# zraorg/ZRA

Measured on AMD Instinct MI355X. Metric: compress + RA-decompress GiB/s, 16 GiB @ 64 KiB frames, 1/2/4/8 MI355X, higher is better.
Workload: dtype u8

## Files before the change

zra_amd/csrc/zra_encode.hip:

```cpp
#include <cstdio>
#include <unistd.h>
#include "zra_engine.h"
#include "zra_dev.h"
#include "zra_format.h"
#include "zra_env.h"
#include <algorithm>
#include <cstdlib>
#include <cstring>
#include <vector>

extern "C" __global__ void zra_mf_kernel(ZraEncArgs a, uint32_t block, uint32_t only, uint32_t onlySlot, uint32_t perWave);
extern "C" __global__ void zra_mf_opt_kernel(ZraEncArgs a, uint32_t block, uint32_t only, uint32_t onlySlot, uint32_t perWave);
extern "C" __global__ void zra_mf_dfast_ls_kernel(ZraEncArgs a, uint32_t block, uint32_t only, uint32_t onlySlot);
extern "C" __global__ void zra_mf_hc_kernel(ZraEncArgs a, uint32_t block, uint32_t only, uint32_t onlySlot);
extern "C" __global__ void zra_mf_fast_kernel(ZraEncArgs a, uint32_t block, uint32_t perWave);
extern "C" __global__ void zra_mf_dfast_kernel(ZraEncArgs a, uint32_t block, uint32_t only, uint32_t onlySlot);
extern "C" __global__ void zra_mf_dfast_fl_kernel(ZraEncArgs a, ZraFlagArgs g, uint32_t block, uint32_t only, uint32_t onlySlot);
extern "C" __global__ void zra_entropy_kernel(ZraEncArgs a, uint32_t block);
extern "C" __global__ void zra_entropy_front_kernel(ZraEncArgs a, uint32_t block);
extern "C" __global__ void zra_entropy_back_kernel(ZraEncArgs a, uint32_t block);
extern "C" __global__ void zra_ent_chain_kernel(ZraEncArgs a);
extern "C" __global__ void zra_ent_chain5_kernel(ZraEncArgs a);

using namespace zra_dev;
// ... 356 lines not shown
  encCounters_ = dCnt; encCountersBytes_ = 4 * (4 + 8 * (size_t)nSuper + 4 * (size_t)(nSuper * subsPerSuper));

  ZraEncArgs base{};
  base.in = dIn; base.inSize = inSize; base.frameSize = frameSize; base.checksum = checksum ? 1 : 0;
  base.full = full; base.tail = tail;
  dbgSeqStride_ = seqStride; dbgB_ = (uint32_t)SBIG;
  base.tableStride = tableWords; base.seqStride = seqStride; base.litStride = litStride; base.slotStride = slotStride;
  base.mfTele = (uint64_t*)(encScan_.as<uint8_t>() + cntCore);
  base.entWorkStride = entWorkStride;
  base.entPrio = 1;
  base.entSubFrames = SB; base.slotRing = (uint32_t)slotRing; base.readyStamp = 1u;
  const uint32_t shL = 1, shS = 3, dupLog = 8;
  base.mfFilter = shL | (shS << 4) | (dupLog << 8);
  const uint32_t hl = std::max(full.hashLog, tail.hashLog), cl = std::max(full.chainLog, tail.chainLog);
  const size_t filterBytes = (8u << dupLog) + (((size_t)1 << hl) >> shL) / 8 + (((size_t)1 << cl) >> shS) / 8;

  static const int lsEnv = env_int("ZRA_MF_LS", 1);
  const uint32_t lsBytes = (uint32_t)((std::min<uint64_t>(frameSize, inSize) + 64 + 63) & ~63ull);
  const uint32_t lsPerCu = (uint32_t)((160u << 10) / (lsBytes + filterBytes));
  static const int lsMaxEnv = env_int("ZRA_MF_LS_MAX", -1);
  bool useLs = lsEnv != 0 && full.strategy == 2 && lsPerCu >= 1 &&
               nFramesTotal <= (lsMaxEnv >= 0 ? (uint64_t)lsMaxEnv : (uint64_t)lsPerCu * (uint64_t)numCUs_);
  if (useLs && lsAttr_ == 0) {
    const bool okA = hipFuncSetAttribute((const void*)zra_mf_dfast_ls_kernel, hipFuncAttributeMaxDynamicSharedMemorySize, 160 << 10) == hipSuccess;
    if (!okA) (void)hipGetLastError();
    lsAttr_ = okA ? 1 : -1;
  }
  if (lsAttr_ < 0) useLs = false;

  static const int flEnv = env_int("ZRA_MF_FLAGS", 1);
  const bool useFlagsWave = flEnv != 0 && !useLs && full.strategy == 2;
  ZraFlagArgs fw{};
  if (useFlagsWave) {
    fw.flagStride = ((((uint64_t)std::min<uint64_t>(frameSize, inSize) + 511) / 512) * 128 + 255) & ~255ull;
    if (!mfFlags_.reserve((size_t)nSlots * fw.flagStride)) return zerr(64);
    fw.flags = mfFlags_.as<uint8_t>(); fw.ldsWords = (uint32_t)(filterBytes / 4);
    fw.spanBytes = 768;
    static const int epEnv = env_int("ZRA_MF_EPOCH", 4);
    const uint32_t ibMax = 32u - (uint32_t)__builtin_clz((uint32_t)std::max<uint64_t>(2, std::min<uint64_t>(frameSize, inSize)) - 1u);
    fw.epochBits = (uint32_t)std::max(0, std::min(epEnv, (int)(32u - ibMax) - 10));
  }
  const size_t spanLds = fw.spanBytes ? fw.spanBytes + 16 + (fw.spanBytes / 64 + 1) * 16 : 0;

  size_t evNext = 0;
  auto ev = [&]() -> hipEvent_t {
    if (evNext == evPool_.size()) { hipEvent_t e = nullptr; if (hipEventCreate(&e) != hipSuccess) return nullptr; evPool_.push_back(e); }
    return evPool_[evNext++];
  };
  std::vector<std::pair<hipEvent_t, hipEvent_t>> mfSpans, entSpans;
  static const bool traceOn = env_set("ZRA_ENC_TRACE");
  hipEvent_t superDone[2] = {nullptr, nullptr};
  { hipEvent_t e0 = ev(); if (!e0) return zerr(1); HIPCHK(hipEventRecord(e0, stream_)); HIPCHK(hipStreamWaitEvent(stream2_, e0, 0)); }

  for (uint64_t S = 0; S < nSuper; S++) {
    const uint64_t F0 = S * SBIG;
    const uint32_t n = (uint32_t)std::min<uint64_t>(SBIG, nFramesTotal - F0);
    const int c = (int)(S % nCtx);
    EncCtx& x = encCtx_[c];
    ZraEncArgs a = base;
    a.firstFrame = (uint32_t)F0; a.nFrames = n;
    a.tables = sh.tables.as<uint32_t>(); a.lits = sh.lits.as<uint8_t>(); a.slots = sh.slots.as<uint8_t>(); a.entWork = sh.work.as<uint8_t>();
    a.seqs = x.seqs.as<uint64_t>();
    a.state = x.misc.as<ZraEncFrameState>();
    a.blockOut = (ZraEncBlockOut*)(x.misc.as<uint8_t>() + (size_t)SBIG * sizeof(ZraEncFrameState));
    a.contentCk = x.ck.as<uint32_t>();
    a.sizes = x.sizes.as<uint64_t>();
    a.mfQueue = dPerSuper + 8 * S; a.mfStarted = a.mfQueue + 1;
    uint32_t* const entQ = dPerSub + 4 * S * subsPerSuper;
    a.mfDone = entQ + 3 * subsPerSuper;
    if (superDone[c]) HIPCHK(hipStreamWaitEvent(stream_, superDone[c], 0));
    HIPCHK(hipMemsetAsync(a.blockOut, 0, (size_t)n * sizeof(ZraEncBlockOut), stream_));
    hipEvent_t m0 = ev(), m1 = ev();
    if (!m0 || !m1) return zerr(1);
    HIPCHK(hipEventRecord(m0, stream_));
    const uint32_t mfGrid = std::min<uint32_t>(n, nSlots);
// ... 209 lines not shown
```

zra_amd/csrc/zra_encode_mf.hip:

```cpp
#include "zra_dev.h"
#include "zra_kernels.h"
#include "zra_encode_wave.h"

using namespace zra_dev;
using namespace zra_wave;

#ifdef ZRA_MF_PROFILE
__device__ unsigned long long zra_mf_prof[24];
#define PROF_DECL u64 pt_[20]; for (int k_ = 0; k_ < 20; k_++) pt_[k_] = 0; u64 pl_ = __builtin_amdgcn_s_memtime();
#define PROF(k) { __builtin_amdgcn_s_waitcnt(0); const u64 n_ = __builtin_amdgcn_s_memtime(); pt_[k] += n_ - pl_; pl_ = n_; }
#define PROF_CNT(k) { pt_[k]++; }
#define PROF_END { if (lane == 0) for (int k_ = 0; k_ < 20; k_++) atomicAdd(&zra_mf_prof[k_], pt_[k_]); }
#elif defined(ZRA_MF_MARK)
#define PROF_DECL
#define PROF(k) asm volatile("; ZMARK " #k);
#define PROF_CNT(k)
#define PROF_END
#else
#define PROF_DECL
#define PROF(k)
#define PROF_CNT(k)
#define PROF_END
#endif

// ... 343 lines not shown
      tS = (((p4 >> ib) & keep) | epoch) << ib;
    }
    if (MLS == 5) bS = (u32)(((v << 24) * 889523592379ULL) >> shS);
    else if (MLS == 6) bS = (u32)(((v << 16) * 227718039650203ULL) >> shS);
    else if (MLS == 7) bS = (u32)(((v << 8) * 58295818150454627ULL) >> shS);
    else bS = p4 >> shS;
  }
};

struct __attribute__((packed, aligned(1))) quad_u { u32 x, y, z, w; };
__device__ __forceinline__ uint4 ld128(const u8* p) { const quad_u q = *(const quad_u*)p; return make_uint4(q.x, q.y, q.z, q.w); }

struct LeanLds {
  u8* dup; u32 dupSlots; u32* bmL; u32* bmS; u32 shL, shS;
  u8* span; u8* spanFlg; u32 spanBytes;
  __device__ __forceinline__ void markL(u32 b) const { const u32 g = b >> shL; atomicOr(&bmL[g >> 5], 1u << (g & 31)); }
  __device__ __forceinline__ void markS(u32 b) const { const u32 g = b >> shS; atomicOr(&bmS[g >> 5], 1u << (g & 31)); }
};

#ifdef ZRA_MF_NT
#define TLD(p) __builtin_nontemporal_load(p)
#define TST(p, v) __builtin_nontemporal_store((u32)(v), p)
#elif defined(ZRA_MF_SC1ST)
#ifdef ZRA_MF_SC1LD
#define TLD(p) __hip_atomic_load((p), __ATOMIC_RELAXED, __HIP_MEMORY_SCOPE_AGENT)
#else
#define TLD(p) (*(p))
#endif
#define TST(p, v) __hip_atomic_store((p), (u32)(v), __ATOMIC_RELAXED, __HIP_MEMORY_SCOPE_AGENT)
#else
#define TLD(p) (*(p))
#define TST(p, v) (*(p) = (v))
#endif
__device__ __forceinline__ u32 df_flags_at(const u8* flg, u32 p) {
  const u8* const w = flg + (size_t)(p >> 6) * 16 + ((p & 63u) >> 3);
  const u32 b = p & 7u;
  return 0x05u | (((w[0] >> b) & 1u) << 1) | (((w[8] >> b) & 1u) << 3);
}
#define ZRA_DF_EPOCH_BITS 4u
template <u32 MLS, bool FLAGS>
__device__ u32 mf_dfast_lean(const ZraEncParams& P, u32* HL, u32* HS, const u8* src, u32 bs, u32 be, u32* rep, u64* seqs, u32* nOut,
                             const LeanLds& W, int lane, u32 ib, const u8* flgIn, u32 epoch = 0) {
  const u8* const flg = FLAGS ? flgIn : nullptr;
  DfHash<MLS, FLAGS ? ZRA_DF_EPOCH_BITS : 0u> H; H.init(P.hashLog, P.chainLog, ib, FLAGS ? rfl(epoch) : 0u);
  const u32 idxMask = ~H.tagMask;
  bs = rfl(bs); be = rfl(be);
  u32 o1 = rfl(rep[0]), o2 = rfl(rep[1]), saved;
  u32 anchor = bs, nseq = 0;
  const u32 ilimit = be >= 8 ? be - 8 : 0;
  u32 ip = mf_prologue(bs, o1, o2, saved);
  u32 sqLo = 0, sqHi = 0;
  u32* const dL = (u32*)W.dup; u32* const dS = dL + W.dupSlots;
  const u32 dmask = W.dupSlots - 1;
  for (u32 i = (u32)lane; i < 2 * W.dupSlots; i += 64) dL[i] = 0;
  u32 dupRound = 0;
  u32* const bmL = W.bmL; u32* const bmS = W.bmS;
  PROF_DECL
  auto emit = [&](u32 ll, u32 ml, u32 offVal) {
    const u64 q = (u64)ll | ((u64)ml << 20) | ((u64)offVal << 40);
    sqLo = wlane(sqLo, (u32)q, nseq & 63); sqHi = wlane(sqHi, (u32)(q >> 32), nseq & 63);
    nseq++;
    if ((nseq & 63) == 0) seqs[nseq - 64 + (u32)lane] = (u64)sqLo | ((u64)sqHi << 32);
  };
  auto insert_slow = [&](u32 pos, bool doL, bool doS) {
    if (lane == 0) {
      const u32 fx = flg ? df_flags_at(flg, pos) : 0x0Fu;
      u32 bl, bs_, tl, ts; H.both(ld64(src + pos), bl, bs_, tl, ts);
      if (doL && (fx & 2)) { TST(HL + bl, (pos + 1) | tl); W.markL(bl); }
      if (doS && (fx & 8)) { TST(HS + bs_, (pos + 1) | ts); W.markS(bs_); }
    }
  };
  const bool useSpan = FLAGS && W.spanBytes != 0;
  u32 sBase = 0, sEnd = 0;
  auto span_fill = [&](u32 at) {
    const u32 mis = (u32)((uintptr_t)(src + at) & 15u);
    const u32 base = rfl(at - min(at, mis));
    const u32 len = min(W.spanBytes, be - base);
    const u32 o = 16u * (u32)lane;
    if (o + 16 <= len) lds_write128(W.span + o, ld128(src + base + o));
    else if (o < len) { for (u32 k = o; k < len; k++) lds_write8(W.span + k, src[base + k]); }
    if (flg) {
      const u32 l2 = (u32)lane, w0 = base >> 6;
      if (l2 <= (W.spanBytes >> 6) && (w0 + l2) * 64u < be) lds_write128(W.spanFlg + 16u * l2, *(const uint4*)(flg + 16u * (size_t)(w0 + l2)));
    }
    __builtin_amdgcn_wave_barrier();
    sBase = base; sEnd = base + len;
  };
  while (ip < ilimit) {
    const u32 wip = ip, run = ip - anchor;
    u32 s = 1, nAct;
    if (run < 256) nAct = min(min(64u, 256u - run), ilimit - ip);
    else { s = (run >> 8) + 1; nAct = min(64u, min((256 * s - run + s - 1) / s, (ilimit - ip + s - 1) / s)); }
    bool active = (u32)lane < nAct;
    const u32 p = wip + (u32)lane * s;
    u64 v8; u32 bflags;
    if (useSpan && s == 1) {
      if (wip < sBase || wip + nAct + 7 > sEnd) span_fill(wip);
      const u32 r = p - sBase;
      v8 = active ? *(const lds_u64u_t*)(W.span + r) : 0;
      bflags = 0x0Fu;
      if (flg && active) {
        const u8* const w = W.spanFlg + ((p >> 6) - (sBase >> 6)) * 16u + ((p & 63u) >> 3);
        const u32 b = p & 7u;
        bflags = 0x05u | (((lds_read8(w) >> b) & 1u) << 1) | (((lds_read8(w + 8) >> b) & 1u) << 3);
      }
    } else {
      v8 = active ? ld64(src + p) : 0;
      bflags = (flg && active) ? df_flags_at(flg, p) : 0x0Fu;
    }
    u32 repFor = o1;
    bool rv = active && o1 > 0 && p + 1 >= o1;
    u32 repVal = rv ? ld32(src + p + 1 - o1) : 0;
    PROF(0) PROF_CNT(12)
    u32 bL, bS, tL, tS; H.both(v8, bL, bS, tL, tS);
    if (nAct > 1) {
      bool pL = active, pS = active;
      u64 mates = 0;
      for (;;) {
        dupRound++;
        const u32 key = (dupRound << 6) | (63u - (u32)lane);
        if (pL) atomicMax(&dL[bL & dmask], key);
        if (pS) atomicMax(&dS[bS & dmask], key);
        __builtin_amdgcn_wave_barrier();
        const u32 wl = pL ? 63u - (lds_read32(&dL[bL & dmask]) & 63u) : (u32)lane;
        const u32 ws = pS ? 63u - (lds_read32(&dS[bS & dmask]) & 63u) : (u32)lane;
        __builtin_amdgcn_wave_barrier();
        const u32 obL = (u32)__shfl((int)bL, (int)wl, 64), obS = (u32)__shfl((int)bS, (int)ws, 64);
        const bool lostL = wl != (u32)lane, lostS = ws != (u32)lane;
        const bool sameL = lostL && obL == bL, sameS = lostS && obS == bS;
        mates |= __ballot(sameL || sameS);
        pL = lostL && !sameL; pS = lostS && !sameS;
        PROF_CNT(17)
        if (!__ballot(pL || pS)) break;
      }
      if (mates) { nAct = (u32)__builtin_ctzll(mates); active = (u32)lane < nAct; }
    }
    PROF(1)
    const u32 gL = bL >> W.shL, gS = bS >> W.shS;
    const u32 wL = gL >> 5, wS = gS >> 5, qL = 1u << (gL & 31), qS = 1u << (gS & 31);
    u32 mL = 0, mS = 0;
    if (active) {
      const bool needL = (bflags & 1) && (bmL[wL] & qL) != 0, needS = (bflags & 4) && (bmS[wS] & qS) != 0;
      const u32 rL = needL ? TLD(HL + bL) : 0u, rS = needS ? TLD(HS + bS) : 0u;
      mL = ((rL & H.tagMask) == tL) ? (rL & idxMask) : 0u;
      mS = ((rS & H.tagMask) == tS) ? (rS & idxMask) : 0u;
    }
    PROF(2)
    u64 LH = __ballot(active && mL > 1);
    u64 SH = __ballot(active && mS > 1);
    const u32 valL = (p + 1) | tL, valS = (p + 1) | tS;
    const u32 v8s = (u32)(v8 >> 8);
    const u64 AM = nAct >= 64 ? ~0ull : (bit64(nAct) - 1);
    u64 RH = __ballot(rv && repVal == v8s);
    u32 repOld = 0, repOldFor = 0xFFFFFFFFu; u64 ROV = 0;
    u64 RV = __ballot(rv);
    PROF(3)
    u32 cur = 0;
    for (;;) {
      if (repFor != o1) {
        rv = active && o1 > 0 && p + 1 >= o1;
        repVal = rv ? ld32(src + p + 1 - o1) : 0; repFor = o1;
        RH = __ballot(rv && repVal == v8s); RV = __ballot(rv);
      }
      const u64 live = AM & (~0ull << cur);
      const u64 hm = (RH | LH | SH) & live;
      if (!hm) {
        if (lane_in(live)) { if (bflags & 2) { TST(HL + bL, valL); atomicOr(&bmL[wL], qL); } if (bflags & 8) { TST(HS + bS, valS); atomicOr(&bmS[wS], qS); } }
        ip = wip + nAct * s; PROF(4)
        break;
      }
      const u32 f = (u32)__builtin_ctzll(hm);
      u64 mkL = live & ((bit64(f) << 1) - 1), mkS = mkL;
      const u32 top = wip + f * s;
      const bool isRep = (RH >> f) & 1, isLong = (LH >> f) & 1;
      ip = top;
      u32 m, known, offVal = 1;
      u32 vneed = 0, mS2 = 0; bool dual = false;
      if (isRep) { ip = top + 1; m = ip - o1; known = 4; }
      else if (isLong) { m = bcast(mL, f) - 1; known = 0; vneed = 8; }
      else if (s == 1 && f + 1 < nAct) {
        mkL |= bit64(f + 1);
        if ((LH >> (f + 1)) & 1) { m = bcast(mL, f + 1) - 1; ip = top + 1; known = 0; vneed = 8; dual = true; mS2 = bcast(mS, f) - 1; }
        else { m = bcast(mS, f) - 1; known = 0; vneed = 4; }
      } else {
        bool hit3; u32 m3;
        {
          PROF_CNT(15)
          if (rfl(ld32(src + bcast(mS, f) - 1)) != bcast((u32)v8, f)) { SH &= ~bit64(f); continue; }
          if (lane_in(mkL) && (bflags & 2)) { TST(HL + bL, valL); atomicOr(&bmL[wL], qL); }
          if (lane_in(mkS) && (bflags & 8)) { TST(HS + bS, valS); atomicOr(&bmS[wS], qS); }
          mkL = 0; mkS = 0;
          u32 m3v = 0; bool h3v = false;
          if (lane == 0) {
            const u64 v9 = ld64(src + top + 1);
            const u32 f3 = flg ? df_flags_at(flg, top + 1) : 0x0Fu;
            u32 b3, bx, t3, tx; H.both(v9, b3, bx, t3, tx);
            const u32 r3 = (f3 & 1) ? TLD(HL + b3) : 0u;
            m3v = ((r3 & H.tagMask) == t3) ? (r3 & idxMask) : 0u;
            if (f3 & 2) { TST(HL + b3, (top + 2) | t3); W.markL(b3); }
            h3v = m3v > 1 && ld64(src + m3v - 1) == v9;
          }
          hit3 = __ballot(h3v) & 1; m3 = bcast(m3v, 0);
        }
        if (hit3) { m = m3 - 1; ip = top + 1; known = 8; }
        else { m = bcast(mS, f) - 1; known = 4; }
      }
      PROF(5)
#ifdef ZRA_MF_PAD_SALU
      { u32 sd_ = nseq;
#pragma unroll
        for (int k_ = 0; k_ < ZRA_MF_PAD_SALU; k_++) asm volatile("s_add_u32 %0, %0, 1" : "+s"(sd_) :: "scc"); }
#endif
#ifdef ZRA_MF_PAD_VALU
      { u32 vd_ = (u32)lane;
#pragma unroll
        for (int k_ = 0; k_ < ZRA_MF_PAD_VALU; k_++) asm volatile("v_add_u32 %0, %0, 1" : "+v"(vd_)); }
#endif
      u32 off = ip - m;
      const u32 l16 = (u32)lane & 15u;
      const bool sec = dual && (u32)lane >= 16 && (u32)lane < 32;
      const u32 fa = sec ? top + 8 * l16 : ip + known + 8 * (u32)lane, fb = sec ? mS2 + 8 * l16 : m + known + 8 * (u32)lane;
      const bool fv = ((u32)lane < 16 || sec) && fa + 8 <= be;
      const u64 xa = fv ? ld64(src + fa) : 0, xb = fv ? ld64(src + fb) : 0;
      const u32 lim = isRep ? 0u : min(ip - anchor, m);
      u32 ya = 0, yb = 1;
      if (lim) { const bool bv = (u32)lane < lim; ya = bv ? src[ip - 1 - lane] : 0u; yb = bv ? src[m - 1 - lane] : 1u; }
      u32 rnext = 0; bool rvn = false;
      if (!isRep) { rvn = active && p + 1 >= off; rnext = rvn ? ld32(src + p + 1 - off) : 0; }
      u32 ml;
      bool redo = false;
      {
        const u64 d = xa ^ xb;
// ... 5 lines not shown
        if (clean) ml = known + 8 * l + bcast(eq, l);
        else ml = known + wave_count_eq(src, ip + known, m + known, be, lane);
        if (dual) {
          const u64 stopS = (stopAll >> 16) & 0xFFFFull;
          const u32 lS = stopS ? (u32)__builtin_ctzll(stopS) : 16u;
          const bool cleanS = stopS && ((fvAll >> (16 + lS)) & 1);
          const u32 mlS = cleanS ? 8 * lS + bcast(eq, 16 + lS) : wave_count_eq(src, top, mS2, be, lane);
          if (mlS < 4) { SH &= ~bit64(f); continue; }
          if (ml < 8) { m = mS2; ip = top; ml = mlS; off = ip - m; redo = true; }
        } else if (ml < vneed) {
          if (isLong) LH &= ~bit64(f); else SH &= ~bit64(f);
          continue;
        }
      }
      PROF(6)
      if (!isRep) {
        u32 back = 0;
        if (redo) {
          back = wave_count_back(src, ip, m, anchor, lane);
          rvn = active && p + 1 >= off; rnext = rvn ? ld32(src + p + 1 - off) : 0;
        } else if (lim) {
          const u64 bad = ~__ballot(ya == yb);
          back = bad ? (u32)__builtin_ctzll(bad) : wave_count_back(src, ip, m, anchor, lane);
        }
        ip -= back; ml += back;
        o2 = o1; o1 = off; offVal = off + 3;
        repOld = repVal; ROV = RV; repOldFor = repFor;
        repVal = rnext; repFor = off; RV = __ballot(rvn); RH = __ballot(rvn && rnext == v8s);
      }
      emit(ip - anchor, ml, offVal);
      ip += ml; anchor = ip;
      PROF(7) PROF_CNT(13)
      if (ip > ilimit) {
        if (lane_in(mkL) && (bflags & 2)) { TST(HL + bL, valL); atomicOr(&bmL[wL], qL); }
        if (lane_in(mkS) && (bflags & 8)) { TST(HS + bS, valS); atomicOr(&bmS[wS], qS); }
        break;
      }
      const u32 relE = ip - wip;
      const bool in2 = s == 1 && f + 2 < nAct;
      const bool inE = s == 1 && relE - 1 < nAct;
      const bool inI = s == 1 && relE < nAct;
      if (in2) { mkL |= bit64(f + 2); mkS |= bit64(f + 2); }
      if (s == 1 && relE - 2 < nAct) mkL |= bit64(relE - 2);
      if (inE) mkS |= bit64(relE - 1);
      if (lane_in(mkL) && (bflags & 2)) { TST(HL + bL, valL); atomicOr(&bmL[wL], qL); }
      if (lane_in(mkS) && (bflags & 8)) { TST(HS + bS, valS); atomicOr(&bmS[wS], qS); }
      u32 here = 0, there = 1;
      const bool thereIn = inI && repOldFor == o2 && ((ROV >> (relE - 1)) & 1);
      if (in2 && inE && (o2 == 0 || thereIn)) {
        if (o2) { here = bcast((u32)v8, relE); there = bcast(repOld, relE - 1); }
      } else {
        PROF_CNT(14)
        const u32 ipos = lane < 2 ? top + 2 : lane == 2 ? ip - 2 : lane == 3 ? ip - 1 : lane == 4 ? ip : ip - o2;
        const u64 x = lane < 6 ? ld64(src + ipos) : 0;
        const u32 fx = (flg && lane < 4) ? df_flags_at(flg, ipos) : 0x0Fu;
        const bool wr = (lane & 1) ? (fx & 8) != 0 : (fx & 2) != 0;
        u32 xbL, xbS, xtL, xtS; H.both(x, xbL, xbS, xtL, xtS);
        u32* const tp = (lane & 1) ? HS + xbS : HL + xbL;
        const u32 tv = (ipos + 1) | ((lane & 1) ? xtS : xtL);
        if (lane < 4 && wr) { if (lane & 1) W.markS(xbS); else W.markL(xbL); }
        if (!in2 && lane < 2 && wr) TST(tp, tv);
        asm volatile("" ::: "memory");
        const u64 later = (s == 1 && relE - 2 < nAct ? 0ull : 4ull) | (inE ? 0ull : 8ull);
        if (lane_in(later) && wr) TST(tp, tv);
        here = bcast((u32)x, 4); there = o2 ? bcast((u32)x, 5) : here + 1;
        if (o2 == 0) { here = 0; there = 1; }
      }
      PROF(8)
      if (here == there) {
        for (;;) {
          PROF_CNT(16)
          const u32 rl = wave_count_eq(src, ip + 4, ip + 4 - o2, be, lane) + 4;
          const u32 t = o2; o2 = o1; o1 = t;
          insert_slow(ip, true, true);
          emit(0, rl, 1);
          ip += rl; anchor = ip;
          if (!(ip <= ilimit && o2 > 0)) break;
          if (rfl(ld32(src + ip)) != rfl(ld32(src + ip - o2))) break;
        }
      }
      PROF(9)
      if (s != 1 || ip >= wip + nAct || ip >= ilimit) break;
      cur = ip - wip;
    }
  }
  if (nseq & 63) { if ((u32)lane < (nseq & 63)) seqs[(nseq & ~63u) + (u32)lane] = (u64)sqLo | ((u64)sqHi << 32); }
  PROF(10) PROF_END
  rep[0] = o1 ? o1 : saved; rep[1] = o2 ? o2 : saved;
  *nOut = nseq;
// ... 326 lines not shown
    O.hashLog3 = P.minMatch == 3 ? min(17u, P.windowLog) : 0;
    O.hash3 = chainT + ((size_t)1 << P.chainLog);
    O.o = (ZraOptState*)(O.hash3 + (O.hashLog3 ? (size_t)1 << O.hashLog3 : 0));
    O.idxShift = st->idxShift;
    ntu = ntu0;
    { const u32 cur = bs + 1 + O.idxShift; if (cur > ntu + 384) { const u32 d = cur - ntu - 384; ntu = cur - (d < 192 ? d : 192); } }
    O.nextToUpdate = ntu;
    if (P.strategy == 9 && O.o->litLengthSum == 0 && bs == 0 && ntu == 1 && be - bs > 1024) {
      u32 tmpRep[3] = {rep[0], rep[1], rep[2]};
      (void)O.parse(src, bs, be, tmpRep, E, true);
      O.idxShift += be - bs;
      O.nextToUpdate = 1 + O.idxShift;
      O.upscale_stats();
    }
    lastLL = O.parse(src, bs, be, rep, E, false);
    ntu = O.nextToUpdate;
    st->idxShift = O.idxShift;
  } else if (P.strategy == 1) lastLL = mf_fast(P, hashT, src, bs, be, rep, E);
  else if (P.strategy == 2) lastLL = mf_dfast_serial(P, hashT, chainT, src, bs, be, rep, E);
  else {
    HC H; H.hashT = hashT; H.chainT = chainT; H.hlog = P.hashLog; H.mls = P.minMatch < 4 ? 4 : P.minMatch > 6 ? 6 : P.minMatch;
    H.chainSize = 1u << P.chainLog; H.cmask = H.chainSize - 1; H.searchLog = P.searchLog; H.nextToUpdate = ntu;
    H.windowLog = P.windowLog;
    H.bt = P.strategy == 6;
    lastLL = mf_lazy(H, src, bs, be, rep, E, P.strategy == 6 ? 2 : (int)P.strategy - 3);
    ntu = H.nextToUpdate;
  }
  st->nextToUpdate = ntu; st->insEnd = ntu;
  bo->nbSeq = E.n; bo->lastLL = lastLL;
  bo->rep[0] = rep[0]; bo->rep[1] = rep[1]; bo->rep[2] = rep[2];
}

struct DfBlock { u64 a; u64 m; };
__device__ __forceinline__ DfBlock df_block_load(const u8* src, u32 fsize, const u8* flg, u32 blk, bool haveMasks, int lane) {
  DfBlock B; B.a = 0; B.m = 0;
  const u32 c = blk * 512 + 8 * (u32)lane;
  if (c + 8 <= fsize) B.a = ld64(src + c);
  else if (c < fsize) B.a = ld64_safe(src + c, src + fsize);
  if (haveMasks && lane < 16) B.m = *(const u64*)(flg + (size_t)blk * 128 + 8 * (u32)lane);
  return B;
}
__device__ __forceinline__ void df_later_flags(const u8* src, u32 fsize, u32 hlog, u32 clog, u32 mls, u32* lds, u32 ldsWords, u8* flg, int lane) {
  if (fsize < 8) return;
  const u32 lastPos = fsize - 8;
  const u32 bmWords = ldsWords - 128;
  u32 npLog = 0;
  while ((((1u << hlog) + (1u << clog)) >> npLog) > bmWords * 32) npLog++;
  const u32 hlogP = hlog - npLog, clogP = clog - npLog;
  u32* const cnt = lds; u32* const bmL = lds + 128; u32* const bmS = bmL + ((1u << hlogP) >> 5);
  const u64 primeS = mls == 5 ? 889523592379ULL : mls == 6 ? 227718039650203ULL : 58295818150454627ULL;
  const u32 shV = 64 - 8 * min(mls, 7u);
  const u32 nBlk = lastPos / 512 + 1;
  const u32 srcLane = (u32)lane >> 3, sh = ((u32)lane & 7u) * 8;
  for (u32 pass = 0; pass < (1u << npLog); pass++) {
    for (u32 i = (u32)lane; i < 128 + ((1u << hlogP) >> 5) + ((1u << clogP) >> 5); i += 64) lds[i] = 0;
    __builtin_amdgcn_fence(__ATOMIC_ACQ_REL, "workgroup");
    const bool hm = pass != 0;
    DfBlock B0 = df_block_load(src, fsize, flg, nBlk - 1, hm, lane), B1{0, 0};
    u64 above = nBlk * 512 < fsize ? ld64_safe(src + nBlk * 512, src + fsize) : 0;
    for (u32 blk = nBlk; blk-- > 0;) {
      if (blk >= 1) B1 = df_block_load(src, fsize, flg, blk - 1, hm, lane);
      const u32 aLo = (u32)B0.a, aHi = (u32)(B0.a >> 32);
      u64 outM = 0;
#pragma unroll 1
      for (u32 kk = 0; kk < 4; kk++) {
        if (blk * 512 + (6 - 2 * kk) * 64 > lastPos) continue;
        u32 iLw[2], iSw[2]; bool pLw[2], pSw[2];
#pragma unroll
        for (int h = 0; h < 2; h++) {
          const u32 k = 7 - 2 * kk - h;
          const u32 p = blk * 512 + k * 64 + (u32)lane;
          const bool act = p <= lastPos;
          const u32 ci = 8 * k + srcLane;
          const u32 c0l = (u32)__builtin_amdgcn_ds_bpermute((int)(4 * ci), (int)aLo), c0h = (u32)__builtin_amdgcn_ds_bpermute((int)(4 * ci), (int)aHi);
          u32 c1l = (u32)__builtin_amdgcn_ds_bpermute((int)(4 * ((ci + 1) & 63)), (int)aLo), c1h = (u32)__builtin_amdgcn_ds_bpermute((int)(4 * ((ci + 1) & 63)), (int)aHi);
          if (ci == 63) { c1l = (u32)above; c1h = (u32)(above >> 32); }
          const u64 c0 = (u64)c0l | ((u64)c0h << 32), c1 = (u64)c1l | ((u64)c1h << 32);
          const u64 v = sh ? (c0 >> sh) | (c1 << (64 - sh)) : c0;
          const u32 bL = (u32)((v * 0xCF1BBCDCB7A56463ULL) >> (64 - hlog));
          const u32 bS = mls <= 4 ? ((u32)v * 2654435761u) >> (32 - clog) : (u32)(((v << shV) * primeS) >> (64 - clog));
          pLw[h] = act && (bL >> hlogP) == pass; pSw[h] = act && (bS >> clogP) == pass;
          iLw[h] = bL & ((1u << hlogP) - 1); iSw[h] = bS & ((1u << clogP) - 1);
        }
        u32 seenL[2], seenS[2], cL[2], cS[2];
#pragma unroll
        for (int h = 0; h < 2; h++) {
          const u32 iL = iLw[h], iS = iSw[h], sL = iL & 255u, sS = 256u + (iS & 255u);
          const bool pL = pLw[h], pS = pSw[h];
          seenL[h] = pL ? lds_read32(&bmL[iL >> 5]) : 0u; seenS[h] = pS ? lds_read32(&bmS[iS >> 5]) : 0u;
          if (pL) atomicAdd(&cnt[sL >> 2], 1u << (8 * (sL & 3)));
          if (pS) atomicAdd(&cnt[sS >> 2], 1u << (8 * (sS & 3)));
          __builtin_amdgcn_wave_barrier();
          cL[h] = pL ? lds_read32(&cnt[sL >> 2]) : 0u;
          cS[h] = pS ? lds_read32(&cnt[sS >> 2]) : 0u;
          __builtin_amdgcn_wave_barrier();
          if (pL) { atomicSub(&cnt[sL >> 2], 1u << (8 * (sL & 3))); atomicOr(&bmL[iL >> 5], 1u << (iL & 31)); }
          if (pS) { atomicSub(&cnt[sS >> 2], 1u << (8 * (sS & 3))); atomicOr(&bmS[iS >> 5], 1u << (iS & 31)); }
          __builtin_amdgcn_wave_barrier();
        }
#pragma unroll
        for (int h = 0; h < 2; h++) {
          const u32 k = 7 - 2 * kk - h;
          if (blk * 512 + k * 64 > lastPos) continue;
          const u32 iL = iLw[h], iS = iSw[h], sL = iL & 255u, sS = iS & 255u;
          const u64 mL = __ballot(((seenL[h] >> (iL & 31)) & 1u) || ((cL[h] >> (8 * (sL & 3))) & 255u) > 1);
          const u64 mS = __ballot(((seenS[h] >> (iS & 31)) & 1u) || ((cS[h] >> (8 * (sS & 3))) & 255u) > 1);
          if ((u32)lane == 2 * k) outM = mL;
          if ((u32)lane == 2 * k + 1) outM = mS;
        }
      }
      if (lane < 16) *(u64*)(flg + (size_t)blk * 128 + 8 * (u32)lane) = outM | B0.m;
      above = (u64)bcast(aLo, 0) | ((u64)bcast(aHi, 0) << 32);
      B0 = B1;
    }
    __builtin_amdgcn_fence(__ATOMIC_RELEASE, "agent");
    __builtin_amdgcn_fence(__ATOMIC_ACQUIRE, "agent");
  }
}
template <bool FLAGS, bool LSRC = false>
__device__ __forceinline__ void mf_dfast_body(const ZraEncArgs& a, u32 block, u32 only, u32 onlySlot, const ZraFlagArgs* g = nullptr) {
  const int lane = threadIdx.x;
  extern __shared__ u32 dynLds[];
  LeanLds W;
  W.shL = a.mfFilter & 15; W.shS = (a.mfFilter >> 4) & 15; W.dupSlots = 1u << ((a.mfFilter >> 8) & 15);
  u32* const fltLds = LSRC ? dynLds + (a.mfFilter >> 16) * 16 : dynLds;
  W.dup = (u8*)fltLds;
  W.bmL = fltLds + 2 * W.dupSlots;
  W.span = nullptr; W.spanFlg = nullptr; W.spanBytes = 0;
  if (FLAGS && g && g->spanBytes) { W.spanBytes = g->spanBytes; W.span = (u8*)(fltLds + g->ldsWords); W.spanFlg = W.span + g->spanBytes + 16; }
  const bool persistent = a.mfQueue != nullptr;
  const bool tele = persistent && a.mfTele != nullptr;
  u64* const tl = tele ? a.mfTele + ZRA_TELE_HEAD + 4 * (size_t)min(blockIdx.x, ZRA_TELE_WAVES - 1u) : nullptr;
  if (tele && lane == 0) {
    const u32 hw = __builtin_amdgcn_s_getreg((31 << 11) | 4);
    const u32 xcc = __builtin_amdgcn_s_getreg((3 << 11) | 20) & 7u;
    const u64 tc0 = __builtin_readcyclecounter(), tr0 = wall_clock64();
    const u32 key = (xcc << 8) | (((hw >> 13) & 7u) << 5) | (((hw >> 12) & 1u) << 4) | ((hw >> 8) & 15u);
    atomicAdd((unsigned long long*)&a.mfTele[32 + key], 1ull << (16u * ((hw >> 4) & 3u)));
    atomicAdd((unsigned long long*)&a.mfTele[8 + xcc], 1ull);
    atomicMax((unsigned long long*)&a.mfTele[4], ~tr0);
    atomicMax((unsigned long long*)&a.mfTele[6], tr0);
    tl[0] = tc0; tl[1] = tr0; tl[2] = xcc; tl[3] = 0;
  }
  if (persistent && a.mfStarted && lane == 0) atomicAdd(a.mfStarted, 1u);
  const u32 epochBits = (FLAGS && g && persistent) ? min(g->epochBits, ZRA_DF_EPOCH_BITS) : 0u;
  u32 epochCtr = 0;
  for (;;) {
    u32 f = only == 0xFFFFFFFFu ? blockIdx.x : only;
    if (persistent) {
      u32 t = 0;
      if (lane == 0) t = atomicAdd(a.mfQueue, 1u);
      f = rfl(t);
      if (f >= a.nFrames) {
        if (tele && lane == 0) {
          const u64 tc1 = __builtin_readcyclecounter(), tr1 = wall_clock64();
          const u64 tc0 = tl[0], tr0 = tl[1];
          const u32 xcc = (u32)tl[2] & 7u;
          atomicAdd((unsigned long long*)&a.mfTele[0], tc1 - tc0);
          atomicAdd((unsigned long long*)&a.mfTele[1], tr1 - tr0);
          atomicAdd((unsigned long long*)&a.mfTele[2], 1ull);
          atomicMax((unsigned long long*)&a.mfTele[3], tr1 - tr0);
          atomicMax((unsigned long long*)&a.mfTele[5], tr1);
// ... 7 lines not shown
    }
#ifdef ZRA_MF_PROFILE
    const u64 kt0_ = __builtin_amdgcn_s_memtime();
#endif
    bool mine = true;
    {
      const u64 fstart = (u64)(a.firstFrame + f) * a.frameSize;
      const ZraEncParams& Pf = (a.inSize - fstart < a.frameSize) ? a.tail : a.full;
      if (Pf.strategy != 2) mine = false;
    }
    MfFrame F;
    bool keepTables = false; u32 epoch = 0;
    if (epochBits && mine) {
      const u64 fstart = (u64)(a.firstFrame + f) * a.frameSize;
      const bool fullFrame = a.inSize - fstart >= a.frameSize;
      if (!fullFrame) epochCtr = 0;
      epoch = epochCtr & ((1u << epochBits) - 1u);
      keepTables = epoch != 0;
      epochCtr = fullFrame ? epochCtr + 1 : 0;
    }
    if (mine && mf_frame_setup(a, block, lane, F, f, persistent ? blockIdx.x : only == 0xFFFFFFFFu ? f : onlySlot, false, keepTables)) {
#ifdef ZRA_MF_PROFILE
      __builtin_amdgcn_s_waitcnt(0);
      if (lane == 0) atomicAdd(&zra_mf_prof[20], __builtin_amdgcn_s_memtime() - kt0_);
#endif
      const u32 wordsL = ((1u << F.P->hashLog) >> W.shL) / 32, wordsS = ((1u << F.P->chainLog) >> W.shS) / 32;
      W.bmS = W.bmL + wordsL;
      u32 rep[3] = {F.st->rep[0], F.st->rep[1], F.st->rep[2]};
      u32 lastLL, nseq = 0;
      const u32 ib = 32 - __builtin_clz(F.fsize - 1);
      const u8* flg = nullptr;
      if (FLAGS && g && g->flags && block == 0 && persistent) {
        u8* const fw = g->flags + (size_t)blockIdx.x * g->flagStride;
        df_later_flags(F.src, F.fsize, F.P->hashLog, F.P->chainLog, F.P->minMatch, fltLds, g->ldsWords, fw, lane);
        flg = fw;
      }
      {
        const u32 fill = block == 0 ? 0u : 0xFFFFFFFFu;
        for (u32 i = lane; i < wordsL + wordsS; i += 64) W.bmL[i] = fill;
        __builtin_amdgcn_fence(__ATOMIC_ACQ_REL, "workgroup");
      }
      const u8* srcP = F.src;
      if (LSRC) {
        u8* const ls = (u8*)dynLds;
        const u32 n16 = F.fsize >> 4;
        for (u32 i = (u32)lane; i < n16; i += 64) *(uint4*)(ls + 16 * i) = ld128(F.src + 16 * i);
        for (u32 i = (n16 << 4) + (u32)lane; i < F.fsize; i += 64) ls[i] = F.src[i];
        ls[F.fsize + (u32)lane] = 0;
        __builtin_amdgcn_fence(__ATOMIC_RELEASE, "workgroup");
        __builtin_amdgcn_wave_barrier();
        __builtin_amdgcn_fence(__ATOMIC_ACQUIRE, "workgroup");
        srcP = ls;
      }
      switch (F.P->minMatch) {
        case 5: lastLL = mf_dfast_lean<5, FLAGS>(*F.P, F.hashT, F.chainT, srcP, F.bs, F.be, rep, F.seqs, &nseq, W, lane, ib, flg, epoch); break;
        case 6: lastLL = mf_dfast_lean<6, FLAGS>(*F.P, F.hashT, F.chainT, srcP, F.bs, F.be, rep, F.seqs, &nseq, W, lane, ib, flg, epoch); break;
        case 7: lastLL = mf_dfast_lean<7, FLAGS>(*F.P, F.hashT, F.chainT, srcP, F.bs, F.be, rep, F.seqs, &nseq, W, lane, ib, flg, epoch); break;
        default: lastLL = mf_dfast_lean<4, FLAGS>(*F.P, F.hashT, F.chainT, srcP, F.bs, F.be, rep, F.seqs, &nseq, W, lane, ib, flg, epoch); break;
      }
      if (lane == 0) {
        F.bo->nbSeq = nseq; F.bo->lastLL = lastLL; F.bo->skip = 0;
        F.bo->rep[0] = rep[0]; F.bo->rep[1] = rep[1]; F.bo->rep[2] = rep[2];
      }
#ifdef ZRA_MF_PROFILE
      __builtin_amdgcn_s_waitcnt(0);
      if (lane == 0) { atomicAdd(&zra_mf_prof[21], __builtin_amdgcn_s_memtime() - kt0_); atomicAdd(&zra_mf_prof[22], 1ull); }
#endif
// ... 114 lines not shown
```

zra_amd/csrc/zra_kernels.h:

```cpp
#pragma once
#include <stdint.h>
#include <stddef.h>

#ifndef ZRA_HUF_FRAMES
#define ZRA_HUF_FRAMES 2
#endif
#define ZRA_DEC_TBL_LL 0u
#define ZRA_DEC_TBL_ML 512u
#define ZRA_DEC_TBL_OF 1024u
#define ZRA_DEC_TBL_WORDS 1280u
#define ZRA_LDS_TBL_LL 0u
#define ZRA_LDS_TBL_ML 1024u
#define ZRA_LDS_TBL_OF 2048u
#define ZRA_LDS_TBL_WORDS 2304u
#define ZRA_CHAIN_LDS_FRAMES 59u
#define ZRA_CHAIN_RING_WORDS 36u

struct ZraDecFrame {
  uint32_t blkPos, produced, done;
  uint32_t hufValid, hufMaxBits, hufNSym, hufX2;
  uint32_t llValid, mlValid, ofValid, llLog, mlLog, ofLog, ofShare;
  uint32_t rep[3];
  uint32_t fcsLo, fcsHi, fcsHave, hasChecksum, bigWindow;
  uint32_t bpos, bsize, blast;
// ... 146 lines not shown
  uint32_t* contentCk;
  uint64_t* sizes;
  uint32_t* mfQueue;
  uint32_t* mfStarted;
  uint32_t* mfDone;
  uint32_t* entQueue;
  uint32_t* entDone;
  uint32_t* scanDone;
  uint32_t* gatherJ;
  uint32_t* gQueue;
  uint32_t* gCopied;
  uint32_t* gatherDone;
  uint32_t* pipeAbort;
  uint64_t* offsets;
  uint64_t* running;
  uint8_t* gBody;
  uint8_t* gEntries;
  uint64_t* gSizesOut;
  uint32_t entSubFrames;
  uint32_t slotRing;
  uint32_t readyStamp;
  uint32_t entPrio;
  uint64_t* mfTele;
  ZraEntRec* entRec;
};
#define ZRA_TELE_CUKEYS 2048u
#define ZRA_TELE_HEAD (32u + ZRA_TELE_CUKEYS)
#define ZRA_TELE_WAVES 8192u
#define ZRA_TELE_ENT (ZRA_TELE_HEAD + 4u * ZRA_TELE_WAVES)
#define ZRA_TELE_WORDS (ZRA_TELE_ENT + 8u + ZRA_TELE_CUKEYS)
struct ZraFlagArgs {
  uint8_t* flags; uint64_t flagStride; uint32_t ldsWords;
  uint32_t spanBytes;
  uint32_t epochBits;
};
```

Measured before the change: 20.37.

## Add forward-pass bucket flags to skip useless hash reads and reuse span LDS

The flag pre-pass now runs in both directions. Besides the existing 'later' bits that gate hash-table writes, it produces 'earlier' bits that gate hash-table reads, which halves the flag stride's density (32 bytes per 64 positions). The match-finder packs the four flag bits into one word per position in LDS and skips global hash loads when no earlier occurrence can exist. Post-match inserts now read bytes and flags from the LDS span instead of global memory, and the span size shrinks. The cost is a second flag pass over each frame and more flag memory traffic, traded against fewer random hash-table reads.

```diff
diff --git a/zra_amd/csrc/zra_encode.hip b/zra_amd/csrc/zra_encode.hip
--- a/zra_amd/csrc/zra_encode.hip
+++ b/zra_amd/csrc/zra_encode.hip
@@ -412,15 +412,20 @@
   const bool useFlagsWave = flEnv != 0 && !useLs && full.strategy == 2;
   ZraFlagArgs fw{};
   if (useFlagsWave) {
-    fw.flagStride = ((((uint64_t)std::min<uint64_t>(frameSize, inSize) + 511) / 512) * 128 + 255) & ~255ull;
+    static const int earlierEnv = env_int("ZRA_MF_EARLIER", 1);
+    fw.earlier = earlierEnv != 0 ? 1u : 0u;
+    fw.flagStride = ((((uint64_t)std::min<uint64_t>(frameSize, inSize) + 511) / 512) * 256 + 255) & ~255ull;
+    static const int spanComplEnv = env_int("ZRA_MF_SPAN_COMPL", 1);
+    fw.spanCompl = spanComplEnv != 0 ? 1u : 0u;
     if (!mfFlags_.reserve((size_t)nSlots * fw.flagStride)) return zerr(64);
     fw.flags = mfFlags_.as<uint8_t>(); fw.ldsWords = (uint32_t)(filterBytes / 4);
-    fw.spanBytes = 768;
+    if (!fw.earlier) HIPCHK(hipMemsetAsync(fw.flags, 0xFF, (size_t)nSlots * fw.flagStride, stream_));
+    fw.spanBytes = 640;
     static const int epEnv = env_int("ZRA_MF_EPOCH", 4);
     const uint32_t ibMax = 32u - (uint32_t)__builtin_clz((uint32_t)std::max<uint64_t>(2, std::min<uint64_t>(frameSize, inSize)) - 1u);
     fw.epochBits = (uint32_t)std::max(0, std::min(epEnv, (int)(32u - ibMax) - 10));
   }
-  const size_t spanLds = fw.spanBytes ? fw.spanBytes + 16 + (fw.spanBytes / 64 + 1) * 16 : 0;
+  const size_t spanLds = fw.spanBytes ? fw.spanBytes + 16 + (fw.spanBytes / 64 + 1) * 32 : 0;
 
   size_t evNext = 0;
   auto ev = [&]() -> hipEvent_t {
diff --git a/zra_amd/csrc/zra_encode_mf.hip b/zra_amd/csrc/zra_encode_mf.hip
--- a/zra_amd/csrc/zra_encode_mf.hip
+++ b/zra_amd/csrc/zra_encode_mf.hip
@@ -399,10 +399,17 @@
 #define TLD(p) (*(p))
 #define TST(p, v) (*(p) = (v))
 #endif
+#define DF_WL 0x00000001u
+#define DF_WS 0x00000100u
+#define DF_RL 0x00010000u
+#define DF_RS 0x01000000u
+#define DF_ALL 0x01010101u
+template <bool EARLIER>
 __device__ __forceinline__ u32 df_flags_at(const u8* flg, u32 p) {
-  const u8* const w = flg + (size_t)(p >> 6) * 16 + ((p & 63u) >> 3);
-  const u32 b = p & 7u;
-  return 0x05u | (((w[0] >> b) & 1u) << 1) | (((w[8] >> b) & 1u) << 3);
+  const u8* const w = flg + (size_t)(p >> 6) * 32 + ((p & 63u) >> 3);
+  u32 d = (u32)w[0] | ((u32)w[8] << 8);
+  if (EARLIER) d |= ((u32)w[16] << 16) | ((u32)w[24] << 24); else d |= 0xFFFF0000u;
+  return (d >> (p & 7u)) & DF_ALL;
 }
 #define ZRA_DF_EPOCH_BITS 4u
 template <u32 MLS, bool FLAGS>
@@ -431,10 +438,10 @@
   };
   auto insert_slow = [&](u32 pos, bool doL, bool doS) {
     if (lane == 0) {
-      const u32 fx = flg ? df_flags_at(flg, pos) : 0x0Fu;
+      const u32 fx = flg ? df_flags_at<false>(flg, pos) : DF_ALL;
       u32 bl, bs_, tl, ts; H.both(ld64(src + pos), bl, bs_, tl, ts);
-      if (doL && (fx & 2)) { TST(HL + bl, (pos + 1) | tl); W.markL(bl); }
-      if (doS && (fx & 8)) { TST(HS + bs_, (pos + 1) | ts); W.markS(bs_); }
+      if (doL && (fx & DF_WL)) { TST(HL + bl, (pos + 1) | tl); W.markL(bl); }
+      if (doS && (fx & DF_WS)) { TST(HS + bs_, (pos + 1) | ts); W.markS(bs_); }
     }
   };
   const bool useSpan = FLAGS && W.spanBytes != 0;
@@ -442,13 +449,18 @@
   auto span_fill = [&](u32 at) {
     const u32 mis = (u32)((uintptr_t)(src + at) & 15u);
     const u32 base = rfl(at - min(at, mis));
-    const u32 len = min(W.spanBytes, be - base);
+    const u32 len = min(W.spanBytes & ~1u, be - base);
     const u32 o = 16u * (u32)lane;
     if (o + 16 <= len) lds_write128(W.span + o, ld128(src + base + o));
     else if (o < len) { for (u32 k = o; k < len; k++) lds_write8(W.span + k, src[base + k]); }
     if (flg) {
       const u32 l2 = (u32)lane, w0 = base >> 6;
-      if (l2 <= (W.spanBytes >> 6) && (w0 + l2) * 64u < be) lds_write128(W.spanFlg + 16u * l2, *(const uint4*)(flg + 16u * (size_t)(w0 + l2)));
+      if (l2 <= (W.spanBytes >> 6) && (w0 + l2) * 64u < be) {
+        const uint4 wl = *(const uint4*)(flg + 32u * (size_t)(w0 + l2)), el = *(const uint4*)(flg + 32u * (size_t)(w0 + l2) + 16);
+        auto mix = [](u32 a, u32 b, u32 c, u32 d, u32 j) { return ((a >> (8 * j)) & 255u) | (((b >> (8 * j)) & 255u) << 8) | (((c >> (8 * j)) & 255u) << 16) | ((d >> (8 * j)) << 24); };
+        lds_write128(W.spanFlg + 32u * l2, make_uint4(mix(wl.x, wl.z, el.x, el.z, 0), mix(wl.x, wl.z, el.x, el.z, 1), mix(wl.x, wl.z, el.x, el.z, 2), mix(wl.x, wl.z, el.x, el.z, 3)));
+        lds_write128(W.spanFlg + 32u * l2 + 16u, make_uint4(mix(wl.y, wl.w, el.y, el.w, 0), mix(wl.y, wl.w, el.y, el.w, 1), mix(wl.y, wl.w, el.y, el.w, 2), mix(wl.y, wl.w, el.y, el.w, 3)));
+      }
     }
     __builtin_amdgcn_wave_barrier();
     sBase = base; sEnd = base + len;
@@ -465,15 +477,11 @@
       if (wip < sBase || wip + nAct + 7 > sEnd) span_fill(wip);
       const u32 r = p - sBase;
       v8 = active ? *(const lds_u64u_t*)(W.span + r) : 0;
-      bflags = 0x0Fu;
-      if (flg && active) {
-        const u8* const w = W.spanFlg + ((p >> 6) - (sBase >> 6)) * 16u + ((p & 63u) >> 3);
-        const u32 b = p & 7u;
-        bflags = 0x05u | (((lds_read8(w) >> b) & 1u) << 1) | (((lds_read8(w + 8) >> b) & 1u) << 3);
-      }
+      bflags = DF_ALL;
+      if (flg && active) bflags = (lds_read32((const u32*)(W.spanFlg + ((p >> 6) - (sBase >> 6)) * 32u + ((p & 63u) >> 3) * 4u)) >> (p & 7u)) & DF_ALL;
     } else {
       v8 = active ? ld64(src + p) : 0;
-      bflags = (flg && active) ? df_flags_at(flg, p) : 0x0Fu;
+      bflags = (flg && active) ? df_flags_at<true>(flg, p) : DF_ALL;
     }
     u32 repFor = o1;
     bool rv = active && o1 > 0 && p + 1 >= o1;
@@ -507,7 +515,7 @@
     const u32 wL = gL >> 5, wS = gS >> 5, qL = 1u << (gL & 31), qS = 1u << (gS & 31);
     u32 mL = 0, mS = 0;
     if (active) {
-      const bool needL = (bflags & 1) && (bmL[wL] & qL) != 0, needS = (bflags & 4) && (bmS[wS] & qS) != 0;
+      const bool needL = (bflags & DF_RL) && (bmL[wL] & qL) != 0, needS = (bflags & DF_RS) && (bmS[wS] & qS) != 0;
       const u32 rL = needL ? TLD(HL + bL) : 0u, rS = needS ? TLD(HS + bS) : 0u;
       mL = ((rL & H.tagMask) == tL) ? (rL & idxMask) : 0u;
       mS = ((rS & H.tagMask) == tS) ? (rS & idxMask) : 0u;
@@ -532,7 +540,7 @@
       const u64 live = AM & (~0ull << cur);
       const u64 hm = (RH | LH | SH) & live;
       if (!hm) {
-        if (lane_in(live)) { if (bflags & 2) { TST(HL + bL, valL); atomicOr(&bmL[wL], qL); } if (bflags & 8) { TST(HS + bS, valS); atomicOr(&bmS[wS], qS); } }
+        if (lane_in(live)) { if (bflags & DF_WL) { TST(HL + bL, valL); atomicOr(&bmL[wL], qL); } if (bflags & DF_WS) { TST(HS + bS, valS); atomicOr(&bmS[wS], qS); } }
         ip = wip + nAct * s; PROF(4)
         break;
       }
@@ -554,17 +562,17 @@
         {
           PROF_CNT(15)
           if (rfl(ld32(src + bcast(mS, f) - 1)) != bcast((u32)v8, f)) { SH &= ~bit64(f); continue; }
-          if (lane_in(mkL) && (bflags & 2)) { TST(HL + bL, valL); atomicOr(&bmL[wL], qL); }
-          if (lane_in(mkS) && (bflags & 8)) { TST(HS + bS, valS); atomicOr(&bmS[wS], qS); }
+          if (lane_in(mkL) && (bflags & DF_WL)) { TST(HL + bL, valL); atomicOr(&bmL[wL], qL); }
+          if (lane_in(mkS) && (bflags & DF_WS)) { TST(HS + bS, valS); atomicOr(&bmS[wS], qS); }
           mkL = 0; mkS = 0;
           u32 m3v = 0; bool h3v = false;
           if (lane == 0) {
             const u64 v9 = ld64(src + top + 1);
-            const u32 f3 = flg ? df_flags_at(flg, top + 1) : 0x0Fu;
+            const u32 f3 = flg ? df_flags_at<true>(flg, top + 1) : DF_ALL;
             u32 b3, bx, t3, tx; H.both(v9, b3, bx, t3, tx);
-            const u32 r3 = (f3 & 1) ? TLD(HL + b3) : 0u;
+            const u32 r3 = (f3 & DF_RL) ? TLD(HL + b3) : 0u;
             m3v = ((r3 & H.tagMask) == t3) ? (r3 & idxMask) : 0u;
-            if (f3 & 2) { TST(HL + b3, (top + 2) | t3); W.markL(b3); }
+            if (f3 & DF_WL) { TST(HL + b3, (top + 2) | t3); W.markL(b3); }
             h3v = m3v > 1 && ld64(src + m3v - 1) == v9;
           }
           hit3 = __ballot(h3v) & 1; m3 = bcast(m3v, 0);
@@ -636,8 +644,8 @@
       ip += ml; anchor = ip;
       PROF(7) PROF_CNT(13)
       if (ip > ilimit) {
-        if (lane_in(mkL) && (bflags & 2)) { TST(HL + bL, valL); atomicOr(&bmL[wL], qL); }
-        if (lane_in(mkS) && (bflags & 8)) { TST(HS + bS, valS); atomicOr(&bmS[wS], qS); }
+        if (lane_in(mkL) && (bflags & DF_WL)) { TST(HL + bL, valL); atomicOr(&bmL[wL], qL); }
+        if (lane_in(mkS) && (bflags & DF_WS)) { TST(HS + bS, valS); atomicOr(&bmS[wS], qS); }
         break;
       }
       const u32 relE = ip - wip;
@@ -647,8 +655,8 @@
       if (in2) { mkL |= bit64(f + 2); mkS |= bit64(f + 2); }
       if (s == 1 && relE - 2 < nAct) mkL |= bit64(relE - 2);
       if (inE) mkS |= bit64(relE - 1);
-      if (lane_in(mkL) && (bflags & 2)) { TST(HL + bL, valL); atomicOr(&bmL[wL], qL); }
-      if (lane_in(mkS) && (bflags & 8)) { TST(HS + bS, valS); atomicOr(&bmS[wS], qS); }
+      if (lane_in(mkL) && (bflags & DF_WL)) { TST(HL + bL, valL); atomicOr(&bmL[wL], qL); }
+      if (lane_in(mkS) && (bflags & DF_WS)) { TST(HS + bS, valS); atomicOr(&bmS[wS], qS); }
       u32 here = 0, there = 1;
       const bool thereIn = inI && repOldFor == o2 && ((ROV >> (relE - 1)) & 1);
       if (in2 && inE && (o2 == 0 || thereIn)) {
@@ -656,9 +664,16 @@
       } else {
         PROF_CNT(14)
         const u32 ipos = lane < 2 ? top + 2 : lane == 2 ? ip - 2 : lane == 3 ? ip - 1 : lane == 4 ? ip : ip - o2;
-        const u64 x = lane < 6 ? ld64(src + ipos) : 0;
-        const u32 fx = (flg && lane < 4) ? df_flags_at(flg, ipos) : 0x0Fu;
-        const bool wr = (lane & 1) ? (fx & 8) != 0 : (fx & 2) != 0;
+        u64 x; u32 fx = DF_ALL;
+        if ((W.spanBytes & 1u) && useSpan && s == 1 && ip + 8 <= sEnd) {
+          PROF_CNT(18)
+          x = lane < 5 ? (u64)*(const lds_u64u_t*)(W.span + (ipos - sBase)) : (lane == 5 && o2) ? ld64(src + ipos) : 0;
+          if (flg && lane < 4) fx = (lds_read32((const u32*)(W.spanFlg + ((ipos >> 6) - (sBase >> 6)) * 32u + ((ipos & 63u) >> 3) * 4u)) >> (ipos & 7u)) & DF_ALL;
+        } else {
+          x = lane < 6 ? ld64(src + ipos) : 0;
+          if (flg && lane < 4) fx = df_flags_at<false>(flg, ipos);
+        }
+        const bool wr = (lane & 1) ? (fx & DF_WS) != 0 : (fx & DF_WL) != 0;
         u32 xbL, xbS, xtL, xtS; H.both(x, xbL, xbS, xtL, xtS);
         u32* const tp = (lane & 1) ? HS + xbS : HL + xbL;
         const u32 tv = (ipos + 1) | ((lane & 1) ? xtS : xtL);
@@ -1051,15 +1066,16 @@
 }
 
 struct DfBlock { u64 a; u64 m; };
-__device__ __forceinline__ DfBlock df_block_load(const u8* src, u32 fsize, const u8* flg, u32 blk, bool haveMasks, int lane) {
+__device__ __forceinline__ DfBlock df_block_load(const u8* src, u32 fsize, const u8* flg, u32 blk, bool haveMasks, u32 dirOff, int lane) {
   DfBlock B; B.a = 0; B.m = 0;
   const u32 c = blk * 512 + 8 * (u32)lane;
   if (c + 8 <= fsize) B.a = ld64(src + c);
   else if (c < fsize) B.a = ld64_safe(src + c, src + fsize);
-  if (haveMasks && lane < 16) B.m = *(const u64*)(flg + (size_t)blk * 128 + 8 * (u32)lane);
+  if (haveMasks && lane < 16) B.m = *(const u64*)(flg + (size_t)blk * 256 + 32 * ((u32)lane >> 1) + 8 * ((u32)lane & 1u) + dirOff);
+  if (lane >= 56 && (blk + 1) * 512 < fsize) { const u32 n = (blk + 1) * 512, at = min(n, fsize - 8); B.m = ld64(src + at) >> (8 * (n - at)); }
   return B;
 }
-__device__ __forceinline__ void df_later_flags(const u8* src, u32 fsize, u32 hlog, u32 clog, u32 mls, u32* lds, u32 ldsWords, u8* flg, int lane) {
+__device__ __forceinline__ void df_bucket_flags(const u8* src, u32 fsize, u32 hlog, u32 clog, u32 mls, u32* lds, u32 ldsWords, u8* flg, bool earlier, int lane) {
   if (fsize < 8) return;
   const u32 lastPos = fsize - 8;
   const u32 bmWords = ldsWords - 128;
@@ -1071,29 +1087,33 @@
   const u32 shV = 64 - 8 * min(mls, 7u);
   const u32 nBlk = lastPos / 512 + 1;
   const u32 srcLane = (u32)lane >> 3, sh = ((u32)lane & 7u) * 8;
-  for (u32 pass = 0; pass < (1u << npLog); pass++) {
+  for (u32 pp = 0; pp < ((earlier ? 2u : 1u) << npLog); pp++) {
+    const u32 pass = pp & ((1u << npLog) - 1u);
+    const bool fwd = (pp >> npLog) != 0;
+    const u32 dirOff = fwd ? 16u : 0u;
     for (u32 i = (u32)lane; i < 128 + ((1u << hlogP) >> 5) + ((1u << clogP) >> 5); i += 64) lds[i] = 0;
     __builtin_amdgcn_fence(__ATOMIC_ACQ_REL, "workgroup");
     const bool hm = pass != 0;
-    DfBlock B0 = df_block_load(src, fsize, flg, nBlk - 1, hm, lane), B1{0, 0};
-    u64 above = nBlk * 512 < fsize ? ld64_safe(src + nBlk * 512, src + fsize) : 0;
-    for (u32 blk = nBlk; blk-- > 0;) {
-      if (blk >= 1) B1 = df_block_load(src, fsize, flg, blk - 1, hm, lane);
+    DfBlock B0 = df_block_load(src, fsize, flg, fwd ? 0u : nBlk - 1, hm, dirOff, lane), B1{0, 0};
+    for (u32 it = 0; it < nBlk; it++) {
+      const u32 blk = fwd ? it : nBlk - 1 - it;
+      if (it + 1 < nBlk) B1 = df_block_load(src, fsize, flg, fwd ? blk + 1 : blk - 1, hm, dirOff, lane);
       const u32 aLo = (u32)B0.a, aHi = (u32)(B0.a >> 32);
       u64 outM = 0;
 #pragma unroll 1
       for (u32 kk = 0; kk < 4; kk++) {
-        if (blk * 512 + (6 - 2 * kk) * 64 > lastPos) continue;
+        const u32 kLow = fwd ? 2 * kk : 6 - 2 * kk;
+        if (blk * 512 + kLow * 64 > lastPos) continue;
         u32 iLw[2], iSw[2]; bool pLw[2], pSw[2];
 #pragma unroll
         for (int h = 0; h < 2; h++) {
-          const u32 k = 7 - 2 * kk - h;
+          const u32 k = kLow + (fwd ? (u32)h : 1u - (u32)h);
           const u32 p = blk * 512 + k * 64 + (u32)lane;
           const bool act = p <= lastPos;
           const u32 ci = 8 * k + srcLane;
           const u32 c0l = (u32)__builtin_amdgcn_ds_bpermute((int)(4 * ci), (int)aLo), c0h = (u32)__builtin_amdgcn_ds_bpermute((int)(4 * ci), (int)aHi);
           u32 c1l = (u32)__builtin_amdgcn_ds_bpermute((int)(4 * ((ci + 1) & 63)), (int)aLo), c1h = (u32)__builtin_amdgcn_ds_bpermute((int)(4 * ((ci + 1) & 63)), (int)aHi);
-          if (ci == 63) { c1l = (u32)above; c1h = (u32)(above >> 32); }
+          if (ci == 63) { c1l = (u32)B0.m; c1h = (u32)(B0.m >> 32); }
           const u64 c0 = (u64)c0l | ((u64)c0h << 32), c1 = (u64)c1l | ((u64)c1h << 32);
           const u64 v = sh ? (c0 >> sh) | (c1 << (64 - sh)) : c0;
           const u32 bL = (u32)((v * 0xCF1BBCDCB7A56463ULL) >> (64 - hlog));
@@ -1119,7 +1139,7 @@
         }
 #pragma unroll
         for (int h = 0; h < 2; h++) {
-          const u32 k = 7 - 2 * kk - h;
+          const u32 k = kLow + (fwd ? (u32)h : 1u - (u32)h);
           if (blk * 512 + k * 64 > lastPos) continue;
           const u32 iL = iLw[h], iS = iSw[h], sL = iL & 255u, sS = iS & 255u;
           const u64 mL = __ballot(((seenL[h] >> (iL & 31)) & 1u) || ((cL[h] >> (8 * (sL & 3))) & 255u) > 1);
@@ -1128,8 +1148,7 @@
           if ((u32)lane == 2 * k + 1) outM = mS;
         }
       }
-      if (lane < 16) *(u64*)(flg + (size_t)blk * 128 + 8 * (u32)lane) = outM | B0.m;
-      above = (u64)bcast(aLo, 0) | ((u64)bcast(aHi, 0) << 32);
+      if (lane < 16) *(u64*)(flg + (size_t)blk * 256 + 32 * ((u32)lane >> 1) + 8 * ((u32)lane & 1u) + dirOff) = outM | B0.m;
       B0 = B1;
     }
     __builtin_amdgcn_fence(__ATOMIC_RELEASE, "agent");
@@ -1146,7 +1165,7 @@
   W.dup = (u8*)fltLds;
   W.bmL = fltLds + 2 * W.dupSlots;
   W.span = nullptr; W.spanFlg = nullptr; W.spanBytes = 0;
-  if (FLAGS && g && g->spanBytes) { W.spanBytes = g->spanBytes; W.span = (u8*)(fltLds + g->ldsWords); W.spanFlg = W.span + g->spanBytes + 16; }
+  if (FLAGS && g && g->spanBytes) { W.spanBytes = g->spanBytes | (g->spanCompl ? 1u : 0u); W.span = (u8*)(fltLds + g->ldsWords); W.spanFlg = W.span + g->spanBytes + 16; }
   const bool persistent = a.mfQueue != nullptr;
   const bool tele = persistent && a.mfTele != nullptr;
   u64* const tl = tele ? a.mfTele + ZRA_TELE_HEAD + 4 * (size_t)min(blockIdx.x, ZRA_TELE_WAVES - 1u) : nullptr;
@@ -1220,7 +1239,7 @@
       const u8* flg = nullptr;
       if (FLAGS && g && g->flags && block == 0 && persistent) {
         u8* const fw = g->flags + (size_t)blockIdx.x * g->flagStride;
-        df_later_flags(F.src, F.fsize, F.P->hashLog, F.P->chainLog, F.P->minMatch, fltLds, g->ldsWords, fw, lane);
+        df_bucket_flags(F.src, F.fsize, F.P->hashLog, F.P->chainLog, F.P->minMatch, fltLds, g->ldsWords, fw, g->earlier != 0, lane);
         flg = fw;
       }
       {
diff --git a/zra_amd/csrc/zra_kernels.h b/zra_amd/csrc/zra_kernels.h
--- a/zra_amd/csrc/zra_kernels.h
+++ b/zra_amd/csrc/zra_kernels.h
@@ -202,5 +202,7 @@
 struct ZraFlagArgs {
   uint8_t* flags; uint64_t flagStride; uint32_t ldsWords;
   uint32_t spanBytes;
+  uint32_t earlier;
+  uint32_t spanCompl;
   uint32_t epochBits;
 };
```

New measurement: 18.61. 0.914x the previous value.
